# lionelblonde/sac-td3-cudagraphs-pytorch

Measured on AMD Instinct MI355X. Metric: gradient-steps/sec (SAC, batch=256) at 1 GPU + 8-seed node; replay HBM GB/s, higher is better.
Workload: dtype f32; 1 GPU; SAC Hopper-v4 batch=256 2x256 MLP+LN, 100000 rows in a 1000000-row HBM ring, 1 critic update+Polyak per iteration, 2 actor+alpha updates every 3rd, hipGraph per 3 iterations; parallelism=1 independent seeds, one per GPU, no collective

## Files before the change

include/sactd3.h:

```cpp
#ifndef SACTD3_H
#define SACTD3_H

#include <stddef.h>
#include <stdint.h>

#ifdef __cplusplus
extern "C" {
#endif

#define SACTD3_ABI_VERSION 1

enum {
  SACTD3_OK = 0,
  SACTD3_EINVAL = -1,
  SACTD3_EHIP = -2,
  SACTD3_ESTATE = -3,
  SACTD3_ENODEV = -4
};

enum {
  SACTD3_ACTOR = 0,
  SACTD3_CRITICS = 1,
  SACTD3_ACTOR_TARGET = 2,
  SACTD3_CRITICS_TARGET = 3,
// ... 37 lines not shown
  int32_t reserved0;
  float actor_lr, qnets_lr, log_alpha_lr;
  float gamma, polyak, alpha_init;
  float clip_norm;
  float td3_std, td3_c, actor_noise_std;
  float adam_beta1, adam_beta2, adam_eps;
  float reserved1;
  uint64_t seed;
} sactd3_config;

typedef struct sactd3_engine sactd3_engine;

void sactd3_default_config(sactd3_config* cfg, int td3);

int sactd3_create(const sactd3_config* cfg, const float* min_ac, const float* max_ac, sactd3_engine** out);
void sactd3_destroy(sactd3_engine* e);
const char* sactd3_last_error(const sactd3_engine* e);
int sactd3_abi_version(void);

int64_t sactd3_param_count(const sactd3_engine* e, int which);
int sactd3_get_params(sactd3_engine* e, int which, float* dst);
int sactd3_set_params(sactd3_engine* e, int which, const float* src);
int sactd3_get_adam_state(sactd3_engine* e, int which, float* exp_avg, float* exp_avg_sq, int64_t* step);
int sactd3_set_adam_state(sactd3_engine* e, int which, const float* exp_avg, const float* exp_avg_sq, int64_t step);

int sactd3_rb_extend(sactd3_engine* e, const float* obs, const float* actions, const float* rewards,
                     const float* next_obs, const uint8_t* dones, int n);
int64_t sactd3_rb_len(const sactd3_engine* e);
int sactd3_rb_layout(const sactd3_engine* e, int32_t out[4]);
int sactd3_rb_extend_device(sactd3_engine* e, const float* records, int n);
typedef struct sactd3_device_fields {
  const float* obs;      int64_t obs_ld;
  const float* actions;  int64_t actions_ld;
  const float* rewards;  int64_t rewards_ld;
  const float* next_obs; int64_t next_obs_ld;
  const uint8_t* dones;  int64_t dones_ld;
} sactd3_device_fields;
#define SACTD3_SRC_ORDERED 1
int sactd3_rb_extend_fields_device(sactd3_engine* e, const sactd3_device_fields* f, int n, void* producer_stream, int flags);
int sactd3_load_batch_device(sactd3_engine* e, const sactd3_device_fields* f, int n, void* producer_stream, int flags);
int sactd3_boundary_stats(const sactd3_engine* e, int64_t out[4]);
typedef struct sactd3_device_fields_out {
  float* obs;      int64_t obs_ld;
  float* actions;  int64_t actions_ld;
  float* rewards;  int64_t rewards_ld;
  float* next_obs; int64_t next_obs_ld;
  uint8_t* dones;  int64_t dones_ld;
  int64_t* index;  int64_t index_ld;
} sactd3_device_fields_out;
#define SACTD3_DST_ORDERED 1
int sactd3_read_batch_device(sactd3_engine* e, const sactd3_device_fields_out* f, void* consumer_stream, int flags);
int sactd3_rb_read_rows_device(sactd3_engine* e, const int64_t* idx, int64_t idx_ld, int n, const sactd3_device_fields_out* f,
                               void* consumer_stream, int flags);
int sactd3_readout_stats(sactd3_engine* e, int64_t out[4]);
int sactd3_rb_sample_indices_device(sactd3_engine* e, const int64_t* idx, int64_t idx_ld, const float* w, int64_t w_ld, int n,
                                    void* caller_stream, int flags );
int sactd3_batch_weights_device(sactd3_engine* e, const float* w, int64_t w_ld, int n, void* caller_stream, int flags );
int sactd3_td_errors_device(sactd3_engine* e, float* td, int64_t td_ld, int64_t td_ns, void* caller_stream, int flags );
int sactd3_priority_stats(sactd3_engine* e, int64_t out[4]);
int sactd3_prio_enable(sactd3_engine* e, float alpha, float eps);
int sactd3_rb_sample_prioritized(sactd3_engine* e, float beta);
int sactd3_prio_set_uniforms(sactd3_engine* e, const float* u, int n);
int sactd3_prio_update_from_td(sactd3_engine* e);
int sactd3_prio_update_device(sactd3_engine* e, const int64_t* idx, int64_t idx_ld, const float* prio, int64_t prio_ld, int n,
                              void* caller_stream, int flags );
int sactd3_prio_stats(sactd3_engine* e, int64_t out[4]);
int sactd3_rb_sample(sactd3_engine* e);
int sactd3_rb_sample_with_indices(sactd3_engine* e, const int64_t* idx, int n);
int sactd3_load_batch(sactd3_engine* e, const float* obs, const float* actions, const float* rewards,
                      const float* next_obs, const uint8_t* dones, int n);
int sactd3_read_batch(sactd3_engine* e, float* obs, float* actions, float* rewards, float* next_obs,
                      uint8_t* dones, int64_t* idx);
int sactd3_rb_fill_synthetic(sactd3_engine* e, int64_t n, uint64_t seed);

int sactd3_set_noise(sactd3_engine* e, int site, const float* eps, int n);
int sactd3_clear_noise(sactd3_engine* e, int site);
int sactd3_read_noise(sactd3_engine* e, int site, float* eps, int n);

int sactd3_update_qnets(sactd3_engine* e);
int sactd3_update_actor(sactd3_engine* e);
int sactd3_update_targ_nets(sactd3_engine* e, int64_t qnet_updates_so_far);
int sactd3_step(sactd3_engine* e, int do_actor);
int sactd3_step_period(sactd3_engine* e);
int sactd3_step_prefix(sactd3_engine* e, int m);
int sactd3_instantiate_graphs(sactd3_engine* e);
int sactd3_predict(sactd3_engine* e, const float* obs, int n, int explore, float* actions);
#define SACTD3_ACT_AFTER_ALL 1
int sactd3_predict_begin(sactd3_engine* e, const float* obs, int n, int explore, int flags);
int sactd3_predict_end(sactd3_engine* e, float* actions);
int sactd3_acting_stats(const sactd3_engine* e, int64_t out[4]);

int sactd3_predict_device(sactd3_engine* e, const float* obs, int64_t obs_ld, int n, int explore,
                          float* actions, int64_t actions_ld, void* caller_stream, int flags);
int sactd3_predict_device_stats(const sactd3_engine* e, int64_t out[4]);

#define SACTD3_Q_ONLINE 0
#define SACTD3_Q_TARGET 1
int sactd3_qvalues_device(sactd3_engine* e, const float* obs, int64_t obs_ld, const float* actions, int64_t actions_ld, int n, int which,
                          float* q, int64_t q_ld, int64_t q_ns, void* caller_stream, int flags );
int sactd3_qvalues(sactd3_engine* e, const float* obs, const float* actions, int n, int which, float* q);
int sactd3_qvalues_stats(const sactd3_engine* e, int64_t out[4]);

int sactd3_read_metrics(sactd3_engine* e, float out[SACTD3_NUM_METRICS]);
int sactd3_device_handles(sactd3_engine* e, void** stream, float** metrics);
int sactd3_sync(sactd3_engine* e);

int64_t sactd3_debug_read(sactd3_engine* e, const char* name, float* dst, int64_t max_floats);
const char* sactd3_debug_names(void);
int sactd3_graph_kernel_count(sactd3_engine* e, int which_graph);
int sactd3_time_kernel(sactd3_engine* e, const char* kernel, int iters, float* usec);
int sactd3_time_nodes(sactd3_engine* e, int do_actor, int iters, int max_nodes, char* names, int names_cap,
                      float* usec, double* flops, double* bytes, int64_t* threads);
int sactd3_time_gather_sweep(sactd3_engine* e, int batch, int iters, float* usec, double* algo_bytes);

#ifdef __cplusplus
}
#endif
#endif
```

sac-td3-cudagraphs-pytorch_amd/_lib.py:

```python
from __future__ import annotations

import ctypes as C
import os
import subprocess

_HERE = os.path.dirname(os.path.abspath(__file__))
_LIB = None

ABI_VERSION = 1
ACTOR, CRITICS, ACTOR_TARGET, CRITICS_TARGET, LOG_ALPHA = range(5)
SITE_CRITIC, SITE_ACTOR0, SITE_ACTOR1, SITE_ALPHA0, SITE_ALPHA1, SITE_PREDICT = range(6)
NUM_METRICS = 8
ACT_AFTER_ALL = 1
SRC_ORDERED = 1
DST_ORDERED = 1
Q_ONLINE, Q_TARGET = 0, 1
ESTATE, EINVAL = -3, -1

SYMBOLS = [
    "sactd3_abi_version", "sactd3_default_config", "sactd3_create", "sactd3_destroy", "sactd3_last_error",
    "sactd3_param_count", "sactd3_get_params", "sactd3_set_params", "sactd3_get_adam_state", "sactd3_set_adam_state",
    "sactd3_rb_extend", "sactd3_rb_len", "sactd3_rb_sample", "sactd3_rb_sample_with_indices", "sactd3_load_batch",
    "sactd3_read_batch", "sactd3_rb_fill_synthetic", "sactd3_set_noise", "sactd3_clear_noise", "sactd3_read_noise",
    "sactd3_update_qnets", "sactd3_update_actor", "sactd3_update_targ_nets", "sactd3_step", "sactd3_predict",
    "sactd3_read_metrics", "sactd3_sync", "sactd3_debug_read", "sactd3_debug_names", "sactd3_graph_kernel_count",
    "sactd3_time_kernel", "sactd3_time_gather_sweep", "sactd3_time_nodes", "sactd3_rb_layout", "sactd3_rb_extend_device", "sactd3_step_period", "sactd3_step_prefix", "sactd3_instantiate_graphs", "sactd3_device_handles",
    "sactd3_predict_begin", "sactd3_predict_end", "sactd3_acting_stats",
    "sactd3_rb_extend_fields_device", "sactd3_load_batch_device", "sactd3_boundary_stats",
    "sactd3_predict_device", "sactd3_predict_device_stats",
    "sactd3_read_batch_device", "sactd3_rb_read_rows_device", "sactd3_readout_stats",
    "sactd3_qvalues_device", "sactd3_qvalues", "sactd3_qvalues_stats",
    "sactd3_rb_sample_indices_device", "sactd3_batch_weights_device", "sactd3_td_errors_device", "sactd3_priority_stats",
    "sactd3_prio_enable", "sactd3_rb_sample_prioritized", "sactd3_prio_set_uniforms", "sactd3_prio_update_from_td", "sactd3_prio_update_device",
    "sactd3_prio_stats",
]


class EngineError(RuntimeError):
    pass


class CConfig(C.Structure):
    _fields_ = [(n, C.c_int32) for n in (
        "abi_version", "ob_dim", "ac_dim", "batch_size", "rb_capacity", "max_envs", "prefer_td3_over_sac",
        "layer_norm", "autotune", "bcq_style_targ_mix", "targ_actor_smoothing", "actor_update_delay",
        "crit_targ_update_freq", "use_graphs", "device_id", "reserved0")] + [(n, C.c_float) for n in (
        "actor_lr", "qnets_lr", "log_alpha_lr", "gamma", "polyak", "alpha_init", "clip_norm", "td3_std", "td3_c",
        "actor_noise_std", "adam_beta1", "adam_beta2", "adam_eps", "reserved1")] + [("seed", C.c_uint64)]


class CDeviceFields(C.Structure):
    _fields_ = [(n, t) for f in ("obs", "actions", "rewards", "next_obs", "dones") for n, t in ((f, C.c_void_p), (f + "_ld", C.c_int64))]


class CDeviceFieldsOut(C.Structure):
    _fields_ = [(n, t) for f in ("obs", "actions", "rewards", "next_obs", "dones", "index") for n, t in ((f, C.c_void_p), (f + "_ld", C.c_int64))]


def library_path() -> str:
    return os.environ.get("SACTD3_LIBRARY") or os.path.join(_HERE, "libsactd3_hip.so")


def build_library(force: bool = False) -> str:
    cmd = ["make", "-C", os.path.join(_HERE, "csrc")] + (["-B"] if force else [])
    subprocess.run(cmd, check=True, stdout=subprocess.PIPE, stderr=subprocess.STDOUT)
    return library_path()


def load_library():
    global _LIB
    if _LIB is not None:
        return _LIB
    path = library_path()
    if not os.path.exists(path):
        raise EngineError(
            f"{path} is missing: build it with `python -c 'import __graft_entry__ as g; g.build()'` "
            "(or `make -C sac-td3-cudagraphs-pytorch_amd/csrc`). There is no CPU fallback.")
    try:
        import torch
    except ImportError:
        pass
    lib = C.CDLL(path)
    fp, u8p, i64p, vp = C.POINTER(C.c_float), C.POINTER(C.c_uint8), C.POINTER(C.c_int64), C.c_void_p
    sig = {
        "sactd3_abi_version": (C.c_int, []),
        "sactd3_default_config": (None, [C.POINTER(CConfig), C.c_int]),
        "sactd3_create": (C.c_int, [C.POINTER(CConfig), fp, fp, C.POINTER(vp)]),
        "sactd3_destroy": (None, [vp]),
        "sactd3_last_error": (C.c_char_p, [vp]),
        "sactd3_param_count": (C.c_int64, [vp, C.c_int]),
        "sactd3_get_params": (C.c_int, [vp, C.c_int, fp]),
        "sactd3_set_params": (C.c_int, [vp, C.c_int, fp]),
        "sactd3_get_adam_state": (C.c_int, [vp, C.c_int, fp, fp, i64p]),
        "sactd3_set_adam_state": (C.c_int, [vp, C.c_int, fp, fp, C.c_int64]),
        "sactd3_rb_extend": (C.c_int, [vp, fp, fp, fp, fp, u8p, C.c_int]),
        "sactd3_rb_len": (C.c_int64, [vp]),
        "sactd3_rb_layout": (C.c_int, [vp, C.POINTER(C.c_int32)]),
        "sactd3_rb_extend_device": (C.c_int, [vp, C.c_void_p, C.c_int]),
        "sactd3_rb_sample": (C.c_int, [vp]),
        "sactd3_rb_sample_with_indices": (C.c_int, [vp, i64p, C.c_int]),
        "sactd3_load_batch": (C.c_int, [vp, fp, fp, fp, fp, u8p, C.c_int]),
        "sactd3_read_batch": (C.c_int, [vp, fp, fp, fp, fp, u8p, i64p]),
        "sactd3_rb_fill_synthetic": (C.c_int, [vp, C.c_int64, C.c_uint64]),
        "sactd3_set_noise": (C.c_int, [vp, C.c_int, fp, C.c_int]),
        "sactd3_clear_noise": (C.c_int, [vp, C.c_int]),
        "sactd3_read_noise": (C.c_int, [vp, C.c_int, fp, C.c_int]),
        "sactd3_update_qnets": (C.c_int, [vp]),
        "sactd3_update_actor": (C.c_int, [vp]),
        "sactd3_update_targ_nets": (C.c_int, [vp, C.c_int64]),
        "sactd3_step": (C.c_int, [vp, C.c_int]),
        "sactd3_step_period": (C.c_int, [vp]),
        "sactd3_step_prefix": (C.c_int, [vp, C.c_int]),
        "sactd3_instantiate_graphs": (C.c_int, [vp]),
        "sactd3_predict": (C.c_int, [vp, fp, C.c_int, C.c_int, fp]),
        "sactd3_predict_begin": (C.c_int, [vp, fp, C.c_int, C.c_int, C.c_int]),
        "sactd3_predict_end": (C.c_int, [vp, fp]),
        "sactd3_acting_stats": (C.c_int, [vp, i64p]),
        "sactd3_rb_extend_fields_device": (C.c_int, [vp, C.POINTER(CDeviceFields), C.c_int, vp, C.c_int]),
        "sactd3_load_batch_device": (C.c_int, [vp, C.POINTER(CDeviceFields), C.c_int, vp, C.c_int]),
        "sactd3_boundary_stats": (C.c_int, [vp, i64p]),
        "sactd3_predict_device": (C.c_int, [vp, vp, C.c_int64, C.c_int, C.c_int, vp, C.c_int64, vp, C.c_int]),
        "sactd3_predict_device_stats": (C.c_int, [vp, i64p]),
        "sactd3_read_batch_device": (C.c_int, [vp, C.POINTER(CDeviceFieldsOut), vp, C.c_int]),
        "sactd3_rb_read_rows_device": (C.c_int, [vp, vp, C.c_int64, C.c_int, C.POINTER(CDeviceFieldsOut), vp, C.c_int]),
        "sactd3_readout_stats": (C.c_int, [vp, i64p]),
        "sactd3_qvalues_device": (C.c_int, [vp, vp, C.c_int64, vp, C.c_int64, C.c_int, C.c_int, vp, C.c_int64, C.c_int64, vp, C.c_int]),
        "sactd3_qvalues": (C.c_int, [vp, fp, fp, C.c_int, C.c_int, fp]),
        "sactd3_qvalues_stats": (C.c_int, [vp, i64p]),
        "sactd3_rb_sample_indices_device": (C.c_int, [vp, vp, C.c_int64, vp, C.c_int64, C.c_int, vp, C.c_int]),
        "sactd3_batch_weights_device": (C.c_int, [vp, vp, C.c_int64, C.c_int, vp, C.c_int]),
        "sactd3_td_errors_device": (C.c_int, [vp, vp, C.c_int64, C.c_int64, vp, C.c_int]),
        "sactd3_priority_stats": (C.c_int, [vp, i64p]),
        "sactd3_prio_enable": (C.c_int, [vp, C.c_float, C.c_float]),
        "sactd3_rb_sample_prioritized": (C.c_int, [vp, C.c_float]),
        "sactd3_prio_set_uniforms": (C.c_int, [vp, fp, C.c_int]),
        "sactd3_prio_update_from_td": (C.c_int, [vp]),
        "sactd3_prio_update_device": (C.c_int, [vp, vp, C.c_int64, vp, C.c_int64, C.c_int, vp, C.c_int]),
        "sactd3_prio_stats": (C.c_int, [vp, i64p]),
        "sactd3_read_metrics": (C.c_int, [vp, fp]),
        "sactd3_sync": (C.c_int, [vp]),
        "sactd3_device_handles": (C.c_int, [vp, C.POINTER(C.c_void_p), C.POINTER(C.c_void_p)]),
        "sactd3_debug_read": (C.c_int64, [vp, C.c_char_p, fp, C.c_int64]),
        "sactd3_debug_names": (C.c_char_p, []),
        "sactd3_graph_kernel_count": (C.c_int, [vp, C.c_int]),
        "sactd3_time_kernel": (C.c_int, [vp, C.c_char_p, C.c_int, fp]),
        "sactd3_time_gather_sweep": (C.c_int, [vp, C.c_int, C.c_int, fp, C.POINTER(C.c_double)]),
        "sactd3_time_nodes": (C.c_int, [vp, C.c_int, C.c_int, C.c_int, C.c_char_p, C.c_int, fp, C.POINTER(C.c_double), C.POINTER(C.c_double), i64p]),
    }
    assert sorted(sig) == sorted(SYMBOLS)
    for name, (res, args) in sig.items():
        fn = getattr(lib, name)
        fn.restype, fn.argtypes = res, args
    if lib.sactd3_abi_version() != ABI_VERSION:
        raise EngineError("libsactd3_hip.so ABI version mismatch; rebuild it")
    _LIB = lib
    return lib
```

sac-td3-cudagraphs-pytorch_amd/csrc/engine.hip:

```cpp
#include <hip/hip_runtime.h>

#include <algorithm>
#include <cmath>
#include <cstdio>
#include <cstdlib>
#include <cstring>
#include <string>
#include <chrono>
#include <vector>

#include "../../include/sactd3.h"
#include "kernels.h"

static thread_local std::string g_create_error;

static inline int round_up(int x, int m) { return (x + m - 1) / m * m; }
static inline unsigned magic_div(unsigned d, unsigned long long n_max) {
  return (d > 1 && n_max * d < (1ull << 32)) ? (unsigned)(((1ull << 32) + d - 1) / d) : 0u;
}

static NetLayout make_layout(int K, int nh) {
  NetLayout L{};
  L.K = K; L.ld1 = round_up(K, 4); L.nh = nh;
  int off = 0;
  L.W1 = off; off += HID * L.ld1;
  L.b1 = off; off += HID; L.g1 = off; off += HID; L.be1 = off; off += HID;
  L.W2 = off; off += HID * HID;
  L.b2 = off; off += HID; L.g2 = off; off += HID; L.be2 = off; off += HID;
  L.Wh = off; off += nh * HID;
  L.bh = off; off += round_up(nh, 4);
  L.size = off;
  return L;
}

static int64_t ref_count(const NetLayout& L, int ln) {
  return (int64_t)HID * L.K + HID + (ln ? 2 * HID : 0) + (int64_t)HID * HID + HID + (ln ? 2 * HID : 0) + (int64_t)L.nh * HID + L.nh;
}
static void pack_net(const NetLayout& L, int ln, const float* src, float* dst, bool is_param) {
  std::fill(dst, dst + L.size, 0.f);
  if (is_param && !ln) {
    std::fill(dst + L.g1, dst + L.g1 + HID, 1.f);
    std::fill(dst + L.g2, dst + L.g2 + HID, 1.f);
  }
  for (int r = 0; r < HID; ++r) { memcpy(dst + L.W1 + (size_t)r * L.ld1, src, sizeof(float) * L.K); src += L.K; }
  memcpy(dst + L.b1, src, sizeof(float) * HID); src += HID;
  if (ln) { memcpy(dst + L.g1, src, sizeof(float) * HID); src += HID; memcpy(dst + L.be1, src, sizeof(float) * HID); src += HID; }
  memcpy(dst + L.W2, src, sizeof(float) * HID * HID); src += HID * HID;
  memcpy(dst + L.b2, src, sizeof(float) * HID); src += HID;
  if (ln) { memcpy(dst + L.g2, src, sizeof(float) * HID); src += HID; memcpy(dst + L.be2, src, sizeof(float) * HID); src += HID; }
  memcpy(dst + L.Wh, src, sizeof(float) * L.nh * HID); src += (size_t)L.nh * HID;
  memcpy(dst + L.bh, src, sizeof(float) * L.nh);
}
static void unpack_net(const NetLayout& L, int ln, const float* src, float* dst) {
  for (int r = 0; r < HID; ++r) { memcpy(dst, src + L.W1 + (size_t)r * L.ld1, sizeof(float) * L.K); dst += L.K; }
  memcpy(dst, src + L.b1, sizeof(float) * HID); dst += HID;
  if (ln) { memcpy(dst, src + L.g1, sizeof(float) * HID); dst += HID; memcpy(dst, src + L.be1, sizeof(float) * HID); dst += HID; }
  memcpy(dst, src + L.W2, sizeof(float) * HID * HID); dst += HID * HID;
  memcpy(dst, src + L.b2, sizeof(float) * HID); dst += HID;
  if (ln) { memcpy(dst, src + L.g2, sizeof(float) * HID); dst += HID; memcpy(dst, src + L.be2, sizeof(float) * HID); dst += HID; }
  memcpy(dst, src + L.Wh, sizeof(float) * L.nh * HID); dst += (size_t)L.nh * HID;
  memcpy(dst, src + L.bh, sizeof(float) * L.nh);
}

static const int BIG_BATCH = 1024;
enum { G_Q = 0, G_A = 1, G_STEP00 = 2, G_STEP01 = 3, G_STEP10 = 4, G_STEP11 = 5, G_PERIOD = 6, G_PERIOD_B = 7, G_OPENING = 8,
       G_PREFIX = 9 ,
       G_QW = 13 , G_COUNT = 14 };
static const int NSTAGE = 32;

struct NodeInfo { std::string name; double flops; double bytes; long threads; };

struct sactd3_engine {
  sactd3_config cfg{};
  std::string err;
  hipStream_t stream = nullptr;
  std::vector<void*> dev_allocs, host_allocs;
  std::vector<hipEvent_t> events;

  int o = 0, a = 0, B = 0, ldc = 0, ldo = 0, a4 = 0, nh = 0, ldu = 0, rec_f = 0, rec4 = 0, cx = 0, cn = 0;
  int nq_actor = 2;
  int nblk = 0, nblk4 = 0;
  int maxn = 0;
  int num_cus = 256;
  int stage_rows = 0;
  NetLayout La{}, Lc{};

  DevCtl* ctl = nullptr;
  float *min_ac = nullptr, *max_ac = nullptr, *scale = nullptr, *bias = nullptr;
  float *Pa = nullptr, *Ta = nullptr, *Ga = nullptr, *Ma = nullptr, *Va = nullptr;
  float *Ta2 = nullptr, *Ta3 = nullptr;
  float *Pc = nullptr, *Tc = nullptr, *Gc = nullptr, *Mc = nullptr, *Vc = nullptr;
  float *la = nullptr, *gscale = nullptr;
  float* ring = nullptr; float* stage_dev = nullptr;
  float *X = nullptr, *Xn = nullptr, *Xp = nullptr, *rew = nullptr, *done = nullptr;
  int* idx = nullptr;
  float *logp_n = nullptr, *logp_pi = nullptr, *logp_al = nullptr, *act_scratch = nullptr;
  float* eps[SACTD3_NUM_SITES] = {};
  float *a_z1 = nullptr, *a_xh1 = nullptr, *a_h1 = nullptr, *a_rs1 = nullptr, *a_z2 = nullptr, *a_xh2 = nullptr, *a_h2 = nullptr, *a_rs2 = nullptr, *a_tg = nullptr;
  float *a_du = nullptr, *a_dz2 = nullptr, *a_dh1 = nullptr, *a_dz1 = nullptr;
  float *qa_ps = nullptr, *qa_S = nullptr;
  float *a_ps = nullptr, *c_ps = nullptr;
  float* a_z2n = nullptr;
  float* ah_z1[4] = {}; float* ah_z2[4] = {};
  struct BatchSlot { float *X, *Xn, *rew, *done, *logp_n, *eps_c; int* idx; float* w; } bs[4] = {};
  int cur_slot = 0;
  int chain_ready = -1;
  bool grads_stale[2] = {false, false};
  float *c_z1 = nullptr, *c_xh1 = nullptr, *c_h1 = nullptr, *c_rs1 = nullptr, *c_z2 = nullptr, *c_dz2 = nullptr, *c_dh1 = nullptr, *c_dz1 = nullptr;
  float *t_z1 = nullptr, *t_z2 = nullptr, *q = nullptr, *qt = nullptr, *y = nullptr, *q_pi = nullptr, *dA = nullptr;
  float* s_h1 = nullptr;
  float* Gp = nullptr; int gp_slabs = 0;
  float *part = nullptr, *part_s = nullptr, *part_sa = nullptr;
  float *p_x = nullptr, *p_z1 = nullptr, *p_z2 = nullptr, *p_act = nullptr;
  float *h_obs = nullptr, *h_act = nullptr;
  int* h_done = nullptr; int predict_calls = 0;
  float* h_stage[NSTAGE] = {}; int stage_next = 0, stage_used = 0;
  float* h_batch = nullptr;

  int64_t rb_len = 0, rb_cursor = 0, qnet_updates = 0;
  hipGraphExec_t graphs[G_COUNT] = {}; int graph_nodes[G_COUNT] = {};
  std::vector<hipGraphExec_t> predict_graphs;
  hipStream_t act_stream = nullptr;
  hipEvent_t ev_learner = nullptr, ev_acting = nullptr;
  bool actor_dirty = true, act_inflight = false, act_ordered = false, act_spin = false;
  int act_n = 0, act_want = 0;
  int64_t act_stats[4] = {};
  hipEvent_t ev_src_ready = nullptr, ev_src_read = nullptr;
  int64_t bnd_stats[4] = {};
  int64_t ro_stats[3] = {};
  long long* time_idx = nullptr;
  std::vector<hipGraphExec_t> predict_dev_graphs;
  int64_t pdev_stats[4] = {};
  float *qs_sa = nullptr, *qs_z1 = nullptr, *qs_z2 = nullptr;
  float *qs_x = nullptr, *qs_az1 = nullptr, *qs_az2 = nullptr, *qs_act = nullptr;
  float *qs_hq = nullptr, *qs_hobs = nullptr, *qs_hact = nullptr;
  int64_t q_stats[4] = {};
  bool slot_weighted = false, td_valid = false;
  int64_t prio_stats[3] = {};
  bool pt_on = false, pt_inject = false;
  float pt_alpha = 0.f, pt_eps = 0.f;
  int pt_groups = 0;
  float *pt_leaf = nullptr, *pt_sums = nullptr, *pt_dleaf = nullptr, *pt_w = nullptr, *pt_total = nullptr, *pt_u = nullptr, *pt_ones = nullptr;
  long long* pt_idx = nullptr;
  struct PrioCtl* pt_ctl = nullptr;
  int64_t pt_host[3] = {};

  int fail(int code, const char* what, hipError_t he = hipSuccess) {
    err = what;
    if (he != hipSuccess) { err += ": "; err += hipGetErrorString(he); }
    return code;
  }
};

#define HIPCHK(call)                                                   \
  do {                                                                 \
    hipError_t _he = (call);                                           \
    if (_he != hipSuccess) return e->fail(SACTD3_EHIP, #call, _he);    \
  } while (0)
#define USE_DEVICE(e)                                                                        \
  do {                                                                                       \
    hipError_t _he = hipSetDevice((e)->cfg.device_id);                                       \
    if (_he != hipSuccess) return (e)->fail(SACTD3_EHIP, "hipSetDevice", _he);               \
    (void)hipGetLastError();    \
  } while (0)
#define CHAIN_BREAK(e) do { (e)->chain_ready = -1; } while (0)
#define SLOT_REFILL(e) do { (e)->slot_weighted = false; (e)->td_valid = false; } while (0)
#define RCCHK(call)                    \
  do {                                 \
    int _rc = (call);                  \
    if (_rc != 0) return _rc;          \
  } while (0)

template <class T>
static int dalloc(sactd3_engine* e, T** p, size_t count, bool zero = true) {
  void* v = nullptr;
  HIPCHK(hipMalloc(&v, std::max<size_t>(count, 4) * sizeof(T)));
  e->dev_allocs.push_back(v);
  if (zero) HIPCHK(hipMemset(v, 0, std::max<size_t>(count, 4) * sizeof(T)));
  *p = (T*)v;
  return 0;
}
template <class T>
static int halloc(sactd3_engine* e, T** p, size_t count) {
  void* v = nullptr;
  HIPCHK(hipHostMalloc(&v, std::max<size_t>(count, 4) * sizeof(T), hipHostMallocDefault));
  e->host_allocs.push_back(v);
  memset(v, 0, std::max<size_t>(count, 4) * sizeof(T));
  *p = (T*)v;
  return 0;
}

struct EnqCtx {
  sactd3_engine* e; hipStream_t s;
  const char* role = "";
  bool lean_stores = false;
  AlphaArgs alpha{}; bool alpha_pending = false;
  bool alpha_tick_owed = false;
  int node_seq = 0, node_only = -1;
  std::vector<NodeInfo>* node_log = nullptr;
};
static int enqueue_end(EnqCtx& x, int rc) {
  return (rc == 0 && (x.alpha_pending || x.alpha_tick_owed)) ? x.e->fail(SACTD3_ESTATE, "enqueue: a deferred temperature step was left over") : rc;
}
// ... 1694 lines not shown
  const float* src = site == SACTD3_SITE_CRITIC ? e->bs[e->cur_slot].eps_c : e->eps[site];
  HIPCHK(hipMemcpy(eps, src, sizeof(float) * (size_t)n * e->a, hipMemcpyDeviceToHost));
  return 0;
}

int sactd3_update_qnets(sactd3_engine* e) {
  if (!e) return SACTD3_EINVAL;
  USE_DEVICE(e);
  CHAIN_BREAK(e);
  e->cur_slot = 0;
  if (e->slot_weighted) {
    IterPlace it;
    it.weighted = true;
    RCCHK(run_graph(e, G_QW, [&](EnqCtx& x) { return enqueue_update_qnets(x, it, false); }));
  } else RCCHK(run_graph(e, G_Q, [&](EnqCtx& x) { return enqueue_update_qnets(x, IterPlace{}, false); }));
  e->grads_stale[0] = false;
  e->td_valid = true;
  return 0;
}
int sactd3_update_actor(sactd3_engine* e) {
  if (!e) return SACTD3_EINVAL;
  USE_DEVICE(e);
  CHAIN_BREAK(e);
  RCCHK(actor_write_begin(e));
  RCCHK(run_graph(e, G_A, [&](EnqCtx& x) { return enqueue_update_actor(x, IterPlace{}, 0, false); }));
  e->grads_stale[1] = false;
  return 0;
}
int sactd3_update_targ_nets(sactd3_engine* e, int64_t qnet_updates_so_far) {
  if (!e) return SACTD3_EINVAL;
  USE_DEVICE(e);
  CHAIN_BREAK(e);
  const bool td3 = e->cfg.prefer_td3_over_sac;
  EnqCtx x{e, e->stream};
  if (td3 || qnet_updates_so_far % e->cfg.crit_targ_update_freq == 0) return enqueue_polyak(x, POLYAK_CRITICS | (td3 ? POLYAK_ACTOR : 0));
  return 0;
}
int sactd3_step(sactd3_engine* e, int do_actor) {
  if (!e) return SACTD3_EINVAL;
  USE_DEVICE(e);
  CHAIN_BREAK(e);
  if (e->rb_len <= 0) return e->fail(SACTD3_ESTATE, "step: buffer is empty");
  const int64_t updates = e->qnet_updates + 1;
  const bool polyak = e->cfg.prefer_td3_over_sac || (updates % e->cfg.crit_targ_update_freq == 0);
  const bool act = do_actor != 0 && e->cfg.actor_update_delay > 0;
  const int which = G_STEP00 + (act ? 2 : 0) + (polyak ? 1 : 0);
  if (act) RCCHK(actor_write_begin(e));
  RCCHK(run_graph(e, which, [&](EnqCtx& x) { return enqueue_step(x, single_iteration(act, polyak)); }));
  e->qnet_updates = updates;
  e->cur_slot = 0;
  e->slot_weighted = false; e->td_valid = true;
  e->grads_stale[0] = false;
  if (act) e->grads_stale[1] = false;
  return 0;
}

static bool actor_dw_is_tiled64(const sactd3_engine* e) {
  return tn_is_tiled64(e, e->B, tn64_tiles(e->nh, HID) + tn64_tiles(HID, HID) + tn64_tiles(HID, e->La.ld1));
}
static bool period_is_pipelined(const sactd3_engine* e) {
  const sactd3_config& c = e->cfg;
  if (c.actor_update_delay < 1 || c.actor_update_delay > 2 || !opening_trunk_gathers(e)) return false;
  if (c.prefer_td3_over_sac) return c.clip_norm <= 0.f && !actor_dw_is_tiled64(e);
  return c.autotune != 0;
}
static void mark_grads_stale(sactd3_engine* e) {
  if (e->cfg.clip_norm > 0.f) return;
  e->grads_stale[0] = true;
  if (e->cfg.actor_update_delay > 0) e->grads_stale[1] = true;
}
static int enqueue_period(EnqCtx& x, int variant, int m) {
  sactd3_engine* e = x.e;
  const bool pipelined = period_is_pipelined(e), whole = m == e->cfg.actor_update_delay + 1;
  x.lean_stores = e->cfg.clip_norm <= 0.f;
  for (int i = 0; i < m; ++i) {
    IterPlace it;
    it.actor = i == 0 && e->cfg.actor_update_delay > 0; it.targets = true; it.more = i + 1 < m;
    if (pipelined) { it.slot = i ? i : (variant ? 3 : 0); it.pre_sampled = true; }
    if (pipelined && i == 0) { it.ahead = m - 1; it.chain_slot = whole ? (variant ? 0 : 3) : -1; }
    RCCHK(enqueue_step(x, it));
  }
  return 0;
}
static int enqueue_opening(EnqCtx& x) {
  if (!opening_merges_policy(x.e)) return x.e->fail(SACTD3_ESTATE, "opening graph: the policy pass did not merge");
  IterPlace it;
  it.actor = true; it.pre_sampled = true;
  return enqueue_opening_pair(x, it, true);
}

int sactd3_step_period(sactd3_engine* e) {
  if (!e) return SACTD3_EINVAL;
  USE_DEVICE(e);
  if (e->rb_len <= 0) return e->fail(SACTD3_ESTATE, "step_period: buffer is empty");
  const bool td3 = e->cfg.prefer_td3_over_sac;
  if (!td3 && e->cfg.crit_targ_update_freq != 1) return e->fail(SACTD3_ESTATE, "step_period: needs crit_targ_update_freq == 1");
  const int n = e->cfg.actor_update_delay + 1;
  RCCHK(actor_write_begin(e));
  mark_grads_stale(e);
  if (!period_is_pipelined(e)) {
    e->chain_ready = -1;
    RCCHK(run_graph(e, G_PERIOD, [&](EnqCtx& x) { return enqueue_period(x, 0, n); }));
    e->cur_slot = 0;
  } else {
    const int v = e->chain_ready >= 0 ? e->chain_ready : 0;
    const bool have = e->chain_ready >= 0;
    e->chain_ready = -1;
    if (!have) RCCHK(run_graph(e, G_OPENING, [&](EnqCtx& x) { return enqueue_opening(x); }));
    RCCHK(run_graph(e, v ? G_PERIOD_B : G_PERIOD, [&](EnqCtx& x) { return enqueue_period(x, v, n); }));
    e->chain_ready = 1 - v;
    e->cur_slot = n - 1;
  }
  e->qnet_updates += n;
  e->slot_weighted = false; e->td_valid = true;
  return 0;
}

int sactd3_step_prefix(sactd3_engine* e, int m) {
  if (!e) return SACTD3_EINVAL;
  USE_DEVICE(e);
  if (m < 1 || m > e->cfg.actor_update_delay) return e->fail(SACTD3_EINVAL, "step_prefix: 1 <= m <= actor_update_delay");
  if (e->rb_len <= 0) return e->fail(SACTD3_ESTATE, "step_prefix: buffer is empty");
  if (!e->cfg.prefer_td3_over_sac && e->cfg.crit_targ_update_freq != 1) return e->fail(SACTD3_ESTATE, "step_prefix: needs crit_targ_update_freq == 1");
  if (!period_is_pipelined(e) || m > 2) {
    for (int i = 0; i < m; ++i) RCCHK(sactd3_step(e, i == 0));
    return 0;
  }
  const int v = e->chain_ready >= 0 ? e->chain_ready : 0;
  const bool have = e->chain_ready >= 0;
  e->chain_ready = -1;
  RCCHK(actor_write_begin(e));
  mark_grads_stale(e);
  if (!have) RCCHK(run_graph(e, G_OPENING, [&](EnqCtx& x) { return enqueue_opening(x); }));
  RCCHK(run_graph(e, G_PREFIX + 2 * (m - 1) + v, [&](EnqCtx& x) { return enqueue_period(x, v, m); }));
  e->cur_slot = m - 1;
  e->qnet_updates += m;
  e->slot_weighted = false; e->td_valid = true;
  return 0;
}

int sactd3_instantiate_graphs(sactd3_engine* e) {
  if (!e) return SACTD3_EINVAL;
  USE_DEVICE(e);
  const bool same_branch = e->cfg.prefer_td3_over_sac || e->cfg.crit_targ_update_freq == 1;
  for (int act = 0; act < 2; ++act)
    for (int pol = same_branch ? 1 : 0; pol < 2; ++pol) {
      const bool a = act != 0 && e->cfg.actor_update_delay > 0, py = pol != 0;
      RCCHK(run_graph(e, G_STEP00 + (a ? 2 : 0) + (py ? 1 : 0), [&](EnqCtx& x) { return enqueue_step(x, single_iteration(a, py)); }, false));
    }
  if (same_branch && e->cfg.actor_update_delay > 0) {
    RCCHK(run_graph(e, G_PERIOD, [&](EnqCtx& x) { return enqueue_period(x, 0, e->cfg.actor_update_delay + 1); }, false));
    if (period_is_pipelined(e)) {
      RCCHK(run_graph(e, G_PERIOD_B, [&](EnqCtx& x) { return enqueue_period(x, 1, e->cfg.actor_update_delay + 1); }, false));
      RCCHK(run_graph(e, G_OPENING, [&](EnqCtx& x) { return enqueue_opening(x); }, false));
      for (int m = 1; m <= e->cfg.actor_update_delay && m <= 2; ++m)
        for (int v = 0; v < 2; ++v)
          RCCHK(run_graph(e, G_PREFIX + 2 * (m - 1) + v, [&](EnqCtx& x) { return enqueue_period(x, v, m); }, false));
    }
  }
  return 0;
}

static bool predict_one_block(sactd3_engine* e, int n) {
  return n <= tail_rows_per_block(tail_args(e, e->p_z2, e->Pa, n, 0, 0, SACTD3_SITE_PREDICT, 48u, e->h_act, e->a4, 0, nullptr));
}
static int enqueue_predict(EnqCtx& x, int n, int explore, bool on_device = false) {
  sactd3_engine* e = x.e;
  const bool td3 = e->cfg.prefer_td3_over_sac;
  bool eps_ready = false;
  {
    const TrunkGrp g{on_device ? e->p_x : e->h_obs, e->Pa, e->p_z1, e->p_z2, nullptr, nullptr, nullptr};
    TrunkTicks tk{nullptr, nullptr, nullptr, nullptr, 0.f};
    if (explore) { tk.nnoise = 1; tk.noise[0] = noise_job(e, SACTD3_SITE_PREDICT, 48u, 0, n); tk.noise_taken = &eps_ready; }
    RCCHK(enqueue_trunk(x, e->ldo, e->o, n, e->La, 0, 1, 1, &g, tk));
  }
  const int mode = td3 ? (explore ? 2 : 0) : (explore ? 0 : 1);
  ActorTail t = tail_args(e, e->p_z2, e->Pa, n, mode, 0, SACTD3_SITE_PREDICT, 48u, on_device ? e->p_act : e->h_act, e->a4, 0, nullptr);
  t.eps_ready = eps_ready;
  const bool one_block = n <= tail_rows_per_block(t);
  if (explore && one_block) t.tick = &e->ctl->predict_ctr;
  if (one_block && !on_device) { t.seq = &e->ctl->predict_seq; t.done_flag = e->h_done; }
  RCCHK(launch_tail(x, t));
  if (explore && !one_block) {
    hipLaunchKernelGGL(k_tick, dim3(1), dim3(1), 0, x.s, &e->ctl->predict_ctr, (int*)nullptr);
    HIPCHK(hipGetLastError());
  }
  return 0;
}
static void predict_stage_obs(sactd3_engine* e, const float* obs, int n) {
  for (int i = 0; i < n; ++i) {
    memset(e->h_obs + (size_t)i * e->ldo, 0, sizeof(float) * e->ldo);
    memcpy(e->h_obs + (size_t)i * e->ldo, obs + (size_t)i * e->o, sizeof(float) * e->o);
  }
}
static int predict_launch(sactd3_engine* e, hipStream_t s, int n, int explore) {
  if (e->predict_graphs.empty()) e->predict_graphs.assign(2 * (size_t)(e->maxn + 1), nullptr);
  return run_graph_slot(e, &e->predict_graphs[(size_t)(explore ? 1 : 0) * (e->maxn + 1) + n], nullptr,
                        [&](EnqCtx& x) { return enqueue_predict(x, n, explore); }, true, s);
}
static int predict_wait(sactd3_engine* e, hipStream_t s, bool spin, int want, bool* by_spin) {
  bool done = false;
  *by_spin = false;
  if (spin) {
    const auto t0 = std::chrono::steady_clock::now();
    for (int spins = 0; !done; ++spins) {
      done = __atomic_load_n(e->h_done, __ATOMIC_ACQUIRE) == want;
      if (!done && (spins & 1023) == 1023 && std::chrono::steady_clock::now() - t0 > std::chrono::milliseconds(2)) break;
    }
    *by_spin = done;
    if (!done) {
      HIPCHK(hipStreamSynchronize(s));
      if (__atomic_load_n(e->h_done, __ATOMIC_ACQUIRE) != want) return e->fail(SACTD3_ESTATE, "predict: the acting kernels did not report completion");
      done = true;
    }
  }
  if (!done) HIPCHK(hipStreamSynchronize(s));
  return 0;
}

int sactd3_predict(sactd3_engine* e, const float* obs, int n, int explore, float* actions) {
  if (!e || !obs || !actions) return SACTD3_EINVAL;
  USE_DEVICE(e);
  if (n < 1 || n > e->maxn) return e->fail(SACTD3_EINVAL, "predict: 1 <= n <= max_envs");
  if (e->act_inflight) return e->fail(SACTD3_ESTATE, "predict: an acting call is in flight (sactd3_predict_end first)");
  predict_stage_obs(e, obs, n);
  RCCHK(predict_launch(e, e->stream, n, explore));
  const bool spin = predict_one_block(e, n);
  bool by_spin = false;
  RCCHK(predict_wait(e, e->stream, spin, spin ? ++e->predict_calls : 0, &by_spin));
  for (int i = 0; i < n; ++i) memcpy(actions + (size_t)i * e->a, e->h_act + (size_t)i * e->a4, sizeof(float) * e->a);
  return 0;
}

int sactd3_predict_begin(sactd3_engine* e, const float* obs, int n, int explore, int flags) {
  if (!e || !obs) return e ? e->fail(SACTD3_EINVAL, "predict_begin: null argument") : SACTD3_EINVAL;
  USE_DEVICE(e);
  if (n < 1 || n > e->maxn) return e->fail(SACTD3_EINVAL, "predict_begin: 1 <= n <= max_envs");
  if (flags & ~SACTD3_ACT_AFTER_ALL) return e->fail(SACTD3_EINVAL, "predict_begin: unknown flag");
  if (e->act_inflight) return e->fail(SACTD3_ESTATE, "predict_begin: an acting call is already in flight (sactd3_predict_end first)");
  if (!e->act_stream) {
    HIPCHK(hipStreamCreateWithFlags(&e->act_stream, hipStreamNonBlocking));
// ... 717 lines not shown
```

sac-td3-cudagraphs-pytorch_amd/engine.py:

```python
from __future__ import annotations

import ctypes as C
from dataclasses import asdict, dataclass
from typing import Dict, Optional

import numpy as np

from . import _lib
from ._lib import EngineError

_F = C.POINTER(C.c_float)


def _f32(x, shape=None) -> np.ndarray:
    arr = np.ascontiguousarray(np.asarray(x, dtype=np.float32))
    if shape is not None:
        arr = arr.reshape(shape)
    return arr


def _fp(a: Optional[np.ndarray]):
    return None if a is None else a.ctypes.data_as(_F)


# ... 186 lines not shown
        self._ck(self.lib.sactd3_boundary_stats(self._h, out))
        return dict(device_extends=int(out[0]), device_rows=int(out[1]), device_batches=int(out[2]), ordered_calls=int(out[3]))

    def _fields_out(self, fields):
        dfo = self._dfo
        ((dfo.obs, dfo.obs_ld), (dfo.actions, dfo.actions_ld), (dfo.rewards, dfo.rewards_ld), (dfo.next_obs, dfo.next_obs_ld),
         (dfo.dones, dfo.dones_ld), (dfo.index, dfo.index_ld)) = [(int(p) or None, int(ld)) for p, ld in fields]
        return C.byref(dfo)

    def read_batch_device(self, fields, consumer_stream: int = 0, ordered: bool = True) -> None:
        self._ck(self.lib.sactd3_read_batch_device(self._h, self._fields_out(fields), C.c_void_p(int(consumer_stream) or None),
                                                   _lib.DST_ORDERED if ordered else 0))

    def rb_read_rows_device(self, idx_ptr: int, idx_ld: int, n: int, fields, consumer_stream: int = 0, ordered: bool = True) -> None:
        self._ck(self.lib.sactd3_rb_read_rows_device(self._h, C.c_void_p(int(idx_ptr) or None), int(idx_ld), int(n), self._fields_out(fields),
                                                     C.c_void_p(int(consumer_stream) or None), _lib.DST_ORDERED if ordered else 0))

    def readout_stats(self) -> Dict[str, int]:
        out = (C.c_int64 * 4)()
        self._ck(self.lib.sactd3_readout_stats(self._h, out))
        return dict(batch_readouts=int(out[0]), row_readouts=int(out[1]), rows_requested=int(out[2]), rows_refused=int(out[3]))

    def rb_len(self) -> int:
        return int(self._ck(self.lib.sactd3_rb_len(self._h)))

    def rb_sample(self) -> None:
        self._ck(self.lib.sactd3_rb_sample(self._h))

    def rb_sample_with_indices(self, idx) -> None:
        idx = np.ascontiguousarray(np.asarray(idx, dtype=np.int64).reshape(-1))
        if idx.size != self.cfg.batch_size:
            raise ValueError(f"expected {self.cfg.batch_size} indices, got {idx.size}")
        self._ck(self.lib.sactd3_rb_sample_with_indices(self._h, idx.ctypes.data_as(C.POINTER(C.c_int64)), idx.size))

    def load_batch(self, obs, act, rew, nobs, done) -> None:
        obs, act, rew, nobs, done, n = self._rows(obs, act, rew, nobs, done)
        self._ck(self.lib.sactd3_load_batch(self._h, _fp(obs), _fp(act), _fp(rew), _fp(nobs),
                                            done.ctypes.data_as(C.POINTER(C.c_uint8)), n))

    def read_batch(self) -> Dict[str, np.ndarray]:
        B, o, a = self.cfg.batch_size, self.cfg.ob_dim, self.cfg.ac_dim
        obs, act = np.empty((B, o), np.float32), np.empty((B, a), np.float32)
        rew, nobs = np.empty(B, np.float32), np.empty((B, o), np.float32)
        done, idx = np.empty(B, np.uint8), np.empty(B, np.int64)
        self._ck(self.lib.sactd3_read_batch(self._h, _fp(obs), _fp(act), _fp(rew), _fp(nobs),
                                            done.ctypes.data_as(C.POINTER(C.c_uint8)),
                                            idx.ctypes.data_as(C.POINTER(C.c_int64))))
        return dict(observations=obs, actions=act, rewards=rew, next_observations=nobs, dones=done.astype(bool), index=idx)

    def rb_fill_synthetic(self, n: int, seed: int = 0) -> None:
        self._ck(self.lib.sactd3_rb_fill_synthetic(self._h, int(n), int(seed)))

    def set_noise(self, site: int, eps) -> None:
        eps = _f32(eps).reshape(-1, self.cfg.ac_dim)
        self._ck(self.lib.sactd3_set_noise(self._h, site, _fp(eps), eps.shape[0]))

    def clear_noise(self, site: int = -1) -> None:
        self._ck(self.lib.sactd3_clear_noise(self._h, site))

    def read_noise(self, site: int, n: Optional[int] = None) -> np.ndarray:
        n = self.cfg.batch_size if n is None else n
        out = np.empty((n, self.cfg.ac_dim), np.float32)
        self._ck(self.lib.sactd3_read_noise(self._h, site, _fp(out), n))
        return out

    def update_qnets(self) -> None:
        self._ck(self.lib.sactd3_update_qnets(self._h))

    def update_actor(self) -> None:
        self._ck(self.lib.sactd3_update_actor(self._h))

    def update_targ_nets(self, qnet_updates_so_far: int) -> None:
        self._ck(self.lib.sactd3_update_targ_nets(self._h, int(qnet_updates_so_far)))

    def step(self, do_actor: bool) -> None:
        self._ck(self.lib.sactd3_step(self._h, int(bool(do_actor))))

    def step_prefix(self, m: int) -> None:
        self._ck(self.lib.sactd3_step_prefix(self._h, int(m)))

    def step_period(self) -> None:
        self._ck(self.lib.sactd3_step_period(self._h))

    def instantiate_graphs(self) -> None:
        self._ck(self.lib.sactd3_instantiate_graphs(self._h))

    def run_iterations(self, i0: int, n: int) -> int:
        period = self.cfg.actor_update_delay + 1
        can = self.cfg.actor_update_delay > 0 and (self.cfg.prefer_td3_over_sac or self.cfg.crit_targ_update_freq == 1)
        i, end = i0, i0 + n
        while i < end:
            if can and i % period == 0 and i + period <= end:
                self.step_period()
                i += period
            elif can and i % period == 0:
                self.step_prefix(end - i)
                i = end
            else:
                self.step(i % period == 0)
                i += 1
        return i

    def predict(self, obs, explore: bool) -> np.ndarray:
        obs = np.asarray(obs)
        n = obs.size // self.cfg.ob_dim
        if 0 < n <= self._st_n and obs.size == n * self.cfg.ob_dim:
            self._st[5][:n] = obs.reshape(n, -1)
            self._ck(self.lib.sactd3_predict(self._h, self._st_p[5], n, 1 if explore else 0, self._st_p[6]))
            return self._st[6][:n].copy()
        obs = _f32(obs).reshape(-1, self.cfg.ob_dim)
        out = np.empty((obs.shape[0], self.cfg.ac_dim), np.float32)
        self._ck(self.lib.sactd3_predict(self._h, _fp(obs), obs.shape[0], int(bool(explore)), _fp(out)))
        return out

    def predict_begin(self, obs, explore: bool, after_all: bool = False) -> None:
        obs = np.asarray(obs)
        n = obs.size // self.cfg.ob_dim
        flags = _lib.ACT_AFTER_ALL if after_all else 0
        if 0 < n <= self._st_n and obs.size == n * self.cfg.ob_dim:
            self._st[5][:n] = obs.reshape(n, -1)
            self._ck(self.lib.sactd3_predict_begin(self._h, self._st_p[5], n, 1 if explore else 0, flags))
        else:
            obs = _f32(obs).reshape(-1, self.cfg.ob_dim)
            n = obs.shape[0]
            self._ck(self.lib.sactd3_predict_begin(self._h, _fp(obs), n, int(bool(explore)), flags))
        self._act_n = n

    def predict_end(self) -> np.ndarray:
        n = getattr(self, "_act_n", 0)
        if 0 < n <= self._st_n:
            self._ck(self.lib.sactd3_predict_end(self._h, self._st_p[6]))
            self._act_n = 0
            return self._st[6][:n].copy()
        out = np.empty((max(n, int(self.cfg.max_envs), 1), self.cfg.ac_dim), np.float32)
        self._ck(self.lib.sactd3_predict_end(self._h, _fp(out)))
        self._act_n = 0
        return out[:n].copy()

    def predict_device(self, obs_ptr: int, obs_ld: int, n: int, explore: bool, out_ptr: int, out_ld: int,
                       caller_stream: int = 0, ordered: bool = True) -> None:
        self._ck(self.lib.sactd3_predict_device(self._h, C.c_void_p(int(obs_ptr) or None), int(obs_ld), int(n), 1 if explore else 0,
                                                C.c_void_p(int(out_ptr) or None), int(out_ld), C.c_void_p(int(caller_stream) or None),
                                                _lib.SRC_ORDERED if ordered else 0))

    def predict_device_stats(self) -> Dict[str, int]:
        out = (C.c_int64 * 4)()
        self._ck(self.lib.sactd3_predict_device_stats(self._h, out))
        return dict(calls=int(out[0]), rows=int(out[1]), ordered_calls=int(out[2]), multi_block_tails=int(out[3]))

    def q_values(self, obs, act=None, target: bool = False) -> np.ndarray:
        obs = _f32(obs).reshape(-1, self.cfg.ob_dim)
        n = obs.shape[0]
        if act is not None:
            act = _f32(act).reshape(-1, self.cfg.ac_dim)
            if act.shape[0] != n:
                raise ValueError(f"observations and actions disagree on the number of rows: {n}, {act.shape[0]}")
        out = np.empty((2, n), np.float32)
        self._ck(self.lib.sactd3_qvalues(self._h, _fp(obs), _fp(act), n, _lib.Q_TARGET if target else _lib.Q_ONLINE, _fp(out)))
        return out

    def q_values_device(self, obs_ptr: int, obs_ld: int, act_ptr: int, act_ld: int, n: int, target: bool, q_ptr: int, q_ld: int,
                        q_ns: int, stream: int = 0, ordered: bool = True) -> None:
        self._ck(self.lib.sactd3_qvalues_device(self._h, C.c_void_p(int(obs_ptr) or None), int(obs_ld), C.c_void_p(int(act_ptr) or None),
                                                int(act_ld), int(n), _lib.Q_TARGET if target else _lib.Q_ONLINE,
                                                C.c_void_p(int(q_ptr) or None), int(q_ld), int(q_ns), C.c_void_p(int(stream) or None),
                                                _lib.SRC_ORDERED if ordered else 0))

    def qvalues_stats(self) -> Dict[str, int]:
        out = (C.c_int64 * 4)()
        self._ck(self.lib.sactd3_qvalues_stats(self._h, out))
        return dict(calls=int(out[0]), rows=int(out[1]), ordered_calls=int(out[2]), policy_calls=int(out[3]))

    def rb_sample_indices_device(self, idx_ptr: int, idx_ld: int, w_ptr: int, w_ld: int, n: int, stream: int = 0, ordered: bool = True) -> None:
        self._ck(self.lib.sactd3_rb_sample_indices_device(self._h, C.c_void_p(int(idx_ptr) or None), int(idx_ld), C.c_void_p(int(w_ptr) or None),
                                                          int(w_ld), int(n), C.c_void_p(int(stream) or None), _lib.SRC_ORDERED if ordered else 0))

    def batch_weights_device(self, w_ptr: int, w_ld: int, n: int, stream: int = 0, ordered: bool = True) -> None:
# ... 86 lines not shown
```

Measured before the change: 19820 gradient-steps/s.

## Batch up to K training periods into one hipGraph launch

Adds multi-period graphs that capture K consecutive 3-iteration periods, alternating the pipelined slot parity, plus a step_periods entry point. run_iterations now issues one call per run of whole periods instead of one per period. This is meant to cut host-side graph launch and Python/ctypes overhead per gradient step. In exchange it instantiates more graphs, which costs memory and setup time, and makes the chain_ready/parity bookkeeping more complex.

```diff
diff --git a/include/sactd3.h b/include/sactd3.h
--- a/include/sactd3.h
+++ b/include/sactd3.h
@@ -143,6 +143,8 @@
 int sactd3_update_targ_nets(sactd3_engine* e, int64_t qnet_updates_so_far);
 int sactd3_step(sactd3_engine* e, int do_actor);
 int sactd3_step_period(sactd3_engine* e);
+int sactd3_step_periods(sactd3_engine* e, int k);
+int sactd3_period_launch_stats(const sactd3_engine* e, int64_t* out, int n);
 int sactd3_step_prefix(sactd3_engine* e, int m);
 int sactd3_instantiate_graphs(sactd3_engine* e);
 int sactd3_predict(sactd3_engine* e, const float* obs, int n, int explore, float* actions);
diff --git a/sac-td3-cudagraphs-pytorch_amd/_lib.py b/sac-td3-cudagraphs-pytorch_amd/_lib.py
--- a/sac-td3-cudagraphs-pytorch_amd/_lib.py
+++ b/sac-td3-cudagraphs-pytorch_amd/_lib.py
@@ -33,6 +33,7 @@
     "sactd3_rb_sample_indices_device", "sactd3_batch_weights_device", "sactd3_td_errors_device", "sactd3_priority_stats",
     "sactd3_prio_enable", "sactd3_rb_sample_prioritized", "sactd3_prio_set_uniforms", "sactd3_prio_update_from_td", "sactd3_prio_update_device",
     "sactd3_prio_stats",
+    "sactd3_step_periods", "sactd3_period_launch_stats",
 ]
 
 
@@ -111,6 +112,8 @@
         "sactd3_step": (C.c_int, [vp, C.c_int]),
         "sactd3_step_period": (C.c_int, [vp]),
         "sactd3_step_prefix": (C.c_int, [vp, C.c_int]),
+        "sactd3_step_periods": (C.c_int, [vp, C.c_int]),
+        "sactd3_period_launch_stats": (C.c_int, [vp, i64p, C.c_int]),
         "sactd3_instantiate_graphs": (C.c_int, [vp]),
         "sactd3_predict": (C.c_int, [vp, fp, C.c_int, C.c_int, fp]),
         "sactd3_predict_begin": (C.c_int, [vp, fp, C.c_int, C.c_int, C.c_int]),
diff --git a/sac-td3-cudagraphs-pytorch_amd/csrc/engine.hip b/sac-td3-cudagraphs-pytorch_amd/csrc/engine.hip
--- a/sac-td3-cudagraphs-pytorch_amd/csrc/engine.hip
+++ b/sac-td3-cudagraphs-pytorch_amd/csrc/engine.hip
@@ -62,10 +62,17 @@
   memcpy(dst, src + L.bh, sizeof(float) * L.nh);
 }
 
+#ifndef SACTD3_MULTI_K
+#define SACTD3_MULTI_K 4
+#endif
+static const int MULTI_K = SACTD3_MULTI_K;
+static_assert(MULTI_K >= 1 && MULTI_K <= 16, "SACTD3_MULTI_K: 1 .. 16 periods per graph");
 static const int BIG_BATCH = 1024;
 enum { G_Q = 0, G_A = 1, G_STEP00 = 2, G_STEP01 = 3, G_STEP10 = 4, G_STEP11 = 5, G_PERIOD = 6, G_PERIOD_B = 7, G_OPENING = 8,
        G_PREFIX = 9 ,
-       G_QW = 13 , G_COUNT = 14 };
+       G_QW = 13 ,
+       G_MULTI = 14 ,
+       G_COUNT = G_MULTI + 2 * (MULTI_K - 1) };
 static const int NSTAGE = 32;
 
 struct NodeInfo { std::string name; double flops; double bytes; long threads; };
@@ -119,6 +126,7 @@
 
   int64_t rb_len = 0, rb_cursor = 0, qnet_updates = 0;
   hipGraphExec_t graphs[G_COUNT] = {}; int graph_nodes[G_COUNT] = {};
+  int64_t period_launches[MULTI_K + 1] = {}, opening_launches = 0;
   std::vector<hipGraphExec_t> predict_graphs;
   hipStream_t act_stream = nullptr;
   hipEvent_t ev_learner = nullptr, ev_acting = nullptr;
@@ -1979,6 +1987,10 @@
   }
   return 0;
 }
+static int enqueue_periods(EnqCtx& x, int v, int m) {
+  for (int j = 0; j < m; ++j) RCCHK(enqueue_period(x, v ^ (j & 1), x.e->cfg.actor_update_delay + 1));
+  return 0;
+}
 static int enqueue_opening(EnqCtx& x) {
   if (!opening_merges_policy(x.e)) return x.e->fail(SACTD3_ESTATE, "opening graph: the policy pass did not merge");
   IterPlace it;
@@ -1986,31 +1998,56 @@
   return enqueue_opening_pair(x, it, true);
 }
 
-int sactd3_step_period(sactd3_engine* e) {
-  if (!e) return SACTD3_EINVAL;
-  USE_DEVICE(e);
-  if (e->rb_len <= 0) return e->fail(SACTD3_ESTATE, "step_period: buffer is empty");
+static int run_periods(sactd3_engine* e, int k, const char* who) {
+  USE_DEVICE(e);
+  auto refuse = [&](const char* what) { e->err = who; e->err += what; return SACTD3_ESTATE; };
+  if (e->rb_len <= 0) return refuse(": buffer is empty");
   const bool td3 = e->cfg.prefer_td3_over_sac;
-  if (!td3 && e->cfg.crit_targ_update_freq != 1) return e->fail(SACTD3_ESTATE, "step_period: needs crit_targ_update_freq == 1");
+  if (!td3 && e->cfg.crit_targ_update_freq != 1) return refuse(": needs crit_targ_update_freq == 1");
   const int n = e->cfg.actor_update_delay + 1;
+  const bool pipelined = period_is_pipelined(e);
   RCCHK(actor_write_begin(e));
   mark_grads_stale(e);
-  if (!period_is_pipelined(e)) {
-    e->chain_ready = -1;
-    RCCHK(run_graph(e, G_PERIOD, [&](EnqCtx& x) { return enqueue_period(x, 0, n); }));
-    e->cur_slot = 0;
-  } else {
-    const int v = e->chain_ready >= 0 ? e->chain_ready : 0;
-    const bool have = e->chain_ready >= 0;
-    e->chain_ready = -1;
-    if (!have) RCCHK(run_graph(e, G_OPENING, [&](EnqCtx& x) { return enqueue_opening(x); }));
-    RCCHK(run_graph(e, v ? G_PERIOD_B : G_PERIOD, [&](EnqCtx& x) { return enqueue_period(x, v, n); }));
-    e->chain_ready = 1 - v;
-    e->cur_slot = n - 1;
-  }
-  e->qnet_updates += n;
-  e->slot_weighted = false; e->td_valid = true;
-  return 0;
+  int v = pipelined && e->chain_ready >= 0 ? e->chain_ready : 0;
+  const bool have = pipelined && e->chain_ready >= 0;
+  e->chain_ready = -1;
+  if (pipelined && !have) {
+    RCCHK(run_graph(e, G_OPENING, [&](EnqCtx& x) { return enqueue_opening(x); }));
+    ++e->opening_launches;
+  }
+  while (k > 0) {
+    const int m = std::min(k, MULTI_K);
+    const int which = m == 1 ? (v ? G_PERIOD_B : G_PERIOD) : G_MULTI + 2 * (m - 2) + v;
+    RCCHK(run_graph(e, which, [&](EnqCtx& x) { return enqueue_periods(x, v, m); }));
+    ++e->period_launches[m];
+    k -= m;
+    e->qnet_updates += (int64_t)m * n;
+    if (pipelined) { v ^= m & 1; e->chain_ready = v; }
+    e->cur_slot = pipelined ? n - 1 : 0;
+    e->slot_weighted = false; e->td_valid = true;
+  }
+  return 0;
+}
+int sactd3_step_period(sactd3_engine* e) {
+  if (!e) return SACTD3_EINVAL;
+  return run_periods(e, 1, "step_period");
+}
+int sactd3_step_periods(sactd3_engine* e, int k) {
+  if (!e) return SACTD3_EINVAL;
+  if (k < 1) return e->fail(SACTD3_EINVAL, "step_periods: k >= 1");
+  return run_periods(e, k, "step_periods");
+}
+int sactd3_period_launch_stats(const sactd3_engine* e, int64_t* out, int n) {
+  if (!e) return SACTD3_EINVAL;
+  const int need = 2 + 2 * MULTI_K;
+  if (!out) return need;
+  if (n < need) return SACTD3_EINVAL;
+  out[0] = MULTI_K; out[1] = e->opening_launches;
+  for (int m = 1; m <= MULTI_K; ++m) {
+    out[1 + m] = e->period_launches[m];
+    out[1 + MULTI_K + m] = m == 1 ? e->graph_nodes[G_PERIOD] : std::max(e->graph_nodes[G_MULTI + 2 * (m - 2)], e->graph_nodes[G_MULTI + 2 * (m - 2) + 1]);
+  }
+  return need;
 }
 
 int sactd3_step_prefix(sactd3_engine* e, int m) {
@@ -2054,6 +2091,9 @@
         for (int v = 0; v < 2; ++v)
           RCCHK(run_graph(e, G_PREFIX + 2 * (m - 1) + v, [&](EnqCtx& x) { return enqueue_period(x, v, m); }, false));
     }
+    for (int m = 2; m <= MULTI_K; ++m)
+      for (int v = 0; v < (period_is_pipelined(e) ? 2 : 1); ++v)
+        RCCHK(run_graph(e, G_MULTI + 2 * (m - 2) + v, [&](EnqCtx& x) { return enqueue_periods(x, v, m); }, false));
   }
   return 0;
 }
diff --git a/sac-td3-cudagraphs-pytorch_amd/engine.py b/sac-td3-cudagraphs-pytorch_amd/engine.py
--- a/sac-td3-cudagraphs-pytorch_amd/engine.py
+++ b/sac-td3-cudagraphs-pytorch_amd/engine.py
@@ -292,17 +292,34 @@
     def step_period(self) -> None:
         self._ck(self.lib.sactd3_step_period(self._h))
 
+    def step_periods(self, k: int) -> None:
+        self._ck(self.lib.sactd3_step_periods(self._h, int(k)))
+
+    def period_launch_stats(self) -> Dict[str, object]:
+        n = int(self._ck(self.lib.sactd3_period_launch_stats(self._h, None, 0)))
+        out = (C.c_int64 * n)()
+        self._ck(self.lib.sactd3_period_launch_stats(self._h, out, n))
+        k = int(out[0])
+        return dict(K=k, opening_launches=int(out[1]), launches={m: int(out[1 + m]) for m in range(1, k + 1)},
+                    nodes={m: int(out[1 + k + m]) for m in range(1, k + 1)})
+
     def instantiate_graphs(self) -> None:
         self._ck(self.lib.sactd3_instantiate_graphs(self._h))
 
     def run_iterations(self, i0: int, n: int) -> int:
         period = self.cfg.actor_update_delay + 1
         can = self.cfg.actor_update_delay > 0 and (self.cfg.prefer_td3_over_sac or self.cfg.crit_targ_update_freq == 1)
+        many = getattr(self, "step_periods", None)
         i, end = i0, i0 + n
         while i < end:
             if can and i % period == 0 and i + period <= end:
-                self.step_period()
-                i += period
+                k = (end - i) // period
+                if many is not None:
+                    many(k)
+                else:
+                    for _ in range(k):
+                        self.step_period()
+                i += k * period
             elif can and i % period == 0:
                 self.step_prefix(end - i)
                 i = end
```

After: 19750 gradient-steps/s. Within noise of the previous version (-0.3%).
